# CVMI-Lab/HybridNeuralRendering

Hardware: AMD Instinct MI355X
Metric: rays/sec (fwd render) scene0241_01 at 1/2/4/8 GPU; PSNR delta vs ref (higher is better)
Workload: dtype f32

## Files before the change

### hybridneuralrendering_amd/csrc/chain_ws.hip

```cpp
#include <utility>

#include "chain_defs.h"
#include "hnr_launch.h"

namespace hnr {

constexpr int CW_CST = ch_lds_exch(4) + 2048;
constexpr int CW_CST_FLOATS = CH_META_DESCALE + 4;
constexpr int CW_DSUM = CW_CST + ((CW_CST_FLOATS * 4 + 15) & ~15);
constexpr int CW_HMAX = CW_DSUM + 4 * 32 * 4 * 4;
constexpr int cw_lds_bytes() { return CW_HMAX + 5 * 512; }

#define CW_LOAD_FRAG(N_, rsrc_, voff_, soff_, IMM_) asm volatile("buffer_load_dwordx4 a[%2:%3], %0, %1, %4 offen offset:%5" :: "v"(voff_), "s"(rsrc_), "n"(N_), "n"((N_) + 3), "s"(soff_), "n"(IMM_))
template <int N> __device__ __forceinline__ void cw_mfma(f32x16 &acc, const u32x4 &x)
{
    asm volatile("v_mfma_f32_32x32x16_f16 %0, a[%2:%3], %1, %0" : "+v"(acc) : "v"(x), "n"(N), "n"(N + 3));
}
template <int N> __device__ __forceinline__ void cw_mfma_first(f32x16 &acc, const u32x4 &x)
{
    asm volatile("v_mfma_f32_32x32x16_f16 %0, a[%2:%3], %1, 0" : "=&v"(acc) : "v"(x), "n"(N), "n"(N + 3));
}
__device__ __forceinline__ void cw_mfma_vw(f32x16 &acc, const u32x4 &w, const u32x4 &x)
{
    asm volatile("v_mfma_f32_32x32x16_f16 %0, %1, %2, %0" : "+v"(acc) : "v"(w), "v"(x));
// ... 31 lines not shown
}

template <class F, int... Is> __device__ __forceinline__ void cw_static_seq(F &&f, std::integer_sequence<int, Is...>) { (f(std::integral_constant<int, Is>{}), ...); }
template <int N, class F> __device__ __forceinline__ void cw_static_for(F &&f) { cw_static_seq(f, std::make_integer_sequence<int, N>{}); }

constexpr int cw_steps(int L) { return L == 0 ? CH_S0 : L == 1 ? CH_S1 : L == 2 ? CH_S2 : CH_S3; }
constexpr int cw_korder(int L, int i) { return L == 1 ? ((i + 8) & 15) : i; }
constexpr int cw_wbase(int L) { return L == 0 ? CH_W0 : L == 1 ? CH_W1 : L == 2 ? CH_W2 : CH_W3; }
constexpr int cw_goff(int P) { int g = 0; for (int p = 0; p < P; ++p) g += cw_steps(p >> 2); return g; }
constexpr int CW_GTOT = cw_goff(16);

constexpr int cw_issue(int P, int slot)
{
    const int L = P >> 2, rt = P & 3;
    if (L == 0) {
        if (rt == 0) return slot == 14 ? 32 + 12 : slot == 20 ? 32 + 13 : -1;
        if (rt == 1) return slot == 17 ? 32 + 14 : -1;
        if (rt == 2) return slot == 17 ? 32 + 15 : -1;
        return -1;
    }
    if (slot % 6 != 5) return -1;
    const int it = slot / 6;
    if (P == 4) return it < 8 ? 32 + it : -1;
    if (P == 7) {
        const int t[16] = {-1, -1, 8, -1, -1, 9, -1, -1, 0, 1, -1, 2, 3, -1, 4, 5};
        return t[it] < 0 ? -1 : 64 + t[it];
    }
    if (P == 8) { const int t[17] = {6, 7, 10, 11, -1, 12, -1, 13, -1, 14, 15, -1, -1, -1, -1, -1, -1}; return t[it] < 0 ? -1 : 64 + t[it]; }
    if (P == 11) return (it & 1) && it < 16 ? 96 + (it >> 1) : -1;
    if (P == 12) { const int t[16] = {8, 9, 10, -1, 11, 12, -1, 13, 14, -1, 15, -1, -1, -1, -1, -1}; return t[it] < 0 ? -1 : 96 + t[it]; }
    if (P == 15) return it < 4 ? it : (it >= 8 && it < 12) ? 32 + it : -1;
    return -1;
}
constexpr int cw_stamp(int P, int slot, int ph) { return (P * 128 + slot) * 4 + ph; }
constexpr int CW_TILE_STAMPS = 16 * 128 * 4;
constexpr int cw_train_stores(int P, int sl)
{
    const int S = cw_steps(P >> 2), T = 6 * S, H = T / 2;
    const bool wide = S == 4;
    int n = 0;
    if (sl < H) {
        const int MS = wide ? 17 : 33, PLe = ((P + 15) & 15) >> 2;
        for (int ms = sl * MS / H; ms < (sl + 1) * MS / H; ++ms) {
            if (wide) { if (ms == 15) n += 4; }
            else if (ms == 23 || ms == 25) n += 2;
            if (ms == MS - 1 && PLe != 3) n += 1;
        }
    } else {
        const int PLe = ((P + 15) & 15) >> 2, MS2 = PLe != 3 ? 21 : 35, k2 = sl - H, N2 = T - H;
        for (int ms = k2 * MS2 / N2; ms < (k2 + 1) * MS2 / N2; ++ms)
            if (ms == 4 || ms == 5) n += 2;
    }
    return n;
}
constexpr int cw_train_stores_pass(int P) { int n = 0; for (int sl = 0; sl < 6 * cw_steps(P >> 2); ++sl) n += cw_train_stores(P, sl); return n; }
static_assert(cw_train_stores_pass(0) == 8 && cw_train_stores_pass(4) == 9 && cw_train_stores_pass(5) == 9 && cw_train_stores_pass(9) == 9 && cw_train_stores_pass(15) == 8, "eight activation stores per pass (+ the sign word of a hidden layer's row tile)");
constexpr int cw_asm_between(int t0, int t1, bool trn = false)
{
    int n = 0;
    for (int wrap = -1; wrap <= 0; ++wrap)
        for (int Q = 0; Q < 16; ++Q)
            for (int sl = 0; sl < 6 * cw_steps(Q >> 2); ++sl) {
                if (cw_issue(Q, sl) >= 0) { const int t = cw_stamp(Q, sl, 2) + wrap * CW_TILE_STAMPS; if (t > t0 && t < t1) n += 4; }
                if ((Q >> 2) == 3 && sl == 3 * cw_steps(3)) { const int t = cw_stamp(Q, sl, 0) + wrap * CW_TILE_STAMPS; if (t > t0 && t < t1) n += 2; }
                if (trn && cw_train_stores(Q, sl) > 0) { const int t = cw_stamp(Q, sl, 3) + wrap * CW_TILE_STAMPS; if (t > t0 && t < t1) n += cw_train_stores(Q, sl); }
            }
    return n;
}
constexpr int cw_need_count(int blk, int P, int slot, bool trn = false)
{
    const int t_need = cw_stamp(P, slot, 1);
    int t_blk = -2 * CW_TILE_STAMPS;
    for (int wrap = -1; wrap <= 0; ++wrap)
        for (int Q = 0; Q < 16; ++Q)
            for (int sl = 0; sl < 6 * cw_steps(Q >> 2); ++sl)
                if (cw_issue(Q, sl) == blk) { const int t = cw_stamp(Q, sl, 2) + wrap * CW_TILE_STAMPS; if (t < t_need && t > t_blk) t_blk = t; }
    return cw_asm_between(t_blk, t_need, trn);
}
constexpr int cw_dma_count(int rt, int Pw, bool trn = false)
{
    const int t1 = cw_stamp(Pw, 3 * cw_steps(Pw >> 2), 0);
    int t0 = cw_stamp(12 + rt, 48, 0);
    if (t0 >= t1) t0 -= CW_TILE_STAMPS;
    return cw_asm_between(t0, t1, trn);
}
static_assert(cw_need_count(32 + 0, 4, 48) == 28 && cw_need_count(32 + 7, 4, 90) == 0, "block1.2's k steps 0..7 are fetched behind the first eight iterations of pass (1,0)");
static_assert(cw_need_count(3, 0, 18) == 22 && cw_need_count(0, 0, 0) == 30, "layer 0 fetches: followed by the image DMA of row tile 3, block1.2's 8..11, then by the first fetch of pass (0,0)");
static_assert(cw_dma_count(3, 2) == 28 && cw_dma_count(0, 15) >= 16, "image DMA waits");

__device__ __forceinline__ void cw_halves(float x, float &lo, float &hi)
{
    const auto r = __builtin_amdgcn_permlane32_swap(__float_as_uint(x), __float_as_uint(x), false, false);
    lo = __uint_as_float(r[0]); hi = __uint_as_float(r[1]);
}
typedef float cw_f32x4 __attribute__((ext_vector_type(4)));
template <class T> using cw_lptr = __attribute__((address_space(3))) T *;
template <int DBG>
__global__ __launch_bounds__(256, 1) void chain_ws_kernel(ChainArgs a)
{
    constexpr bool TR = DBG == 8;
    constexpr int DB = TR ? 0 : DBG;
    constexpr int SLOT = ch_slot(4);
    extern __shared__ __attribute__((aligned(16))) char lds[];
    const int tid = threadIdx.x, lane = tid & 63, wave = __builtin_amdgcn_readfirstlane(tid >> 6), h = lane >> 5, j = lane & 31;
    const ChainClasses cls = chain_classes(a.counts, a.cap_samples);
    const int n_valid = cls.n_valid, n_tiles = cls.n_tiles;
    const float *meta = reinterpret_cast<const float *>(a.wimg + CH_META);
    const __amdgpu_buffer_rsrc_t wsrd = __builtin_amdgcn_make_buffer_rsrc(const_cast<char *>(a.wimg), 0, CH_WBYTES, 0x00020000);
    const int col0 = 64 * wave + 16 * h;
    const unsigned woff = (unsigned)(2 * wave) * 2048u + (unsigned)lane * 16u;
    const int o_b0 = (int)lane * 16, o_b1 = o_b0 + 65536, o_b2 = o_b0 + 131072;
    const int o_pub = (int)(4 * wave + h) * SLOT + (int)j * 16;
    const int o_ext = 16 * SLOT + (int)j * 16;
    const int o_exw = (int)ch_lds_exch(4) + (int)(j * 4 + wave) * 4, o_exr = (int)ch_lds_exch(4) + (int)j * 16;
    const int o_dsw = (int)CW_DSUM + (int)(j * 4 + wave) * 4, o_dsr = (int)CW_DSUM + (int)wave * 512 + (int)j * 16;
    const int o_cst = (int)CW_CST + (int)col0 * 4;
#define CW_KEEP(x_) ({ int k_ = (x_); asm volatile("" : "+v"(k_)); k_; })
#define CW_LDS(T_, off_) (*reinterpret_cast<T_ *>(lds + (off_)))
#define CW_AT(T_, ptr_, off_) (*reinterpret_cast<cw_lptr<T_>>((ptr_) + (off_)))
// ... 9 lines not shown
        if constexpr (pe_ != 3) { q_pub = CW_KEEPP(p_pub); q_exw = CW_KEEPP(p_exw); q_exr = CW_KEEPP(p_exr); } \
        if constexpr (pe_ == 1) q_ext = CW_KEEPP(p_ext); \
        if constexpr (pe_ == 3) { q_dsw = CW_KEEPP(p_dsw); q_dsr = CW_KEEPP(p_dsr); } } while (0)

    const int xcd = blockIdx.x & 7, nb = (gridDim.x + 7 - xcd) / 8, bi = blockIdx.x >> 3;
    const int per = (n_tiles + 7) / 8, t_lo = xcd * per, t_hi = (t_lo + per < n_tiles) ? t_lo + per : n_tiles;
    const bool xcd_order = gridDim.x >= 8;
    const int t_first = xcd_order ? t_lo + bi : (int)blockIdx.x, t_end = xcd_order ? t_hi : n_tiles, t_step = xcd_order ? nb : (int)gridDim.x;
    if (t_first >= t_end) return;

    for (int i = tid; i < 2 * 4 * 32; i += 256)
        CW_LDS(u32x4, 16 * SLOT + (i >> 5) * 1024 + (32 + (i & 31)) * 16) = u32x4{0u, 0u, 0u, 0u};
    for (int i = tid; i < CW_CST_FLOATS; i += 256) CW_LDS(float, CW_CST + 4 * i) = meta[i];
    if constexpr (TR) { for (int i = tid; i < 5 * 128; i += 256) CW_LDS(float, CW_HMAX + 4 * i) = 0.f; }

    asm volatile("" ::: "a255");
    u32x4 wx[2][2];
    f32x16 acc[2][2];
    u32x4 bf[3][2];
    float inv[4] = {0.f, 0.f, 0.f, 0.f};
    int pid[4], pid_n[4] = {0, 0, 0, 0};
    float wq[4], wq_fin = 0.f;
    float4 e0 = make_float4(0.f, 0.f, 0.f, 0.f), e1 = e0;
    float4 tv[TR ? 1 : 2][2][4];
#define CW_TV(i_) tv[TR ? 0 : ((i_) & 1)]

#ifndef HNR_CHAIN_WS_SAME_W
#define HNR_CHAIN_WS_SAME_W 0
#endif
#define CW_LOAD_W(L_, s_) do { \
        const int so_ = cw_wbase(L_) + (HNR_CHAIN_WS_SAME_W ? 0 : (s_)) * CH_WSTEP; \
        CW_LOAD_FRAG(16 * (s_) + 0, wsrd, woff, so_, 0); CW_LOAD_FRAG(16 * (s_) + 4, wsrd, woff, so_, 1024); \
        CW_LOAD_FRAG(16 * (s_) + 8, wsrd, woff, so_, 2048); CW_LOAD_FRAG(16 * (s_) + 12, wsrd, woff, so_, 3072); } while (0)
    auto load_ids = [&](int tile, int (&pd)[4]) __attribute__((always_inline)) {
        const char *aux = a.aux + (size_t)tile * 4 * CH_AUX_GROUP;
#pragma unroll
        for (int rt = 0; rt < 4; ++rt) {
            if constexpr (TR) { const int u = a.row_u[(size_t)tile * 128 + 32 * rt + j]; pd[rt] = (unsigned)u >= (unsigned)a.ucap ? 0 : u; }
            else pd[rt] = reinterpret_cast<const int32_t *>(aux + rt * CH_AUX_GROUP)[j];
        }
    };
    auto load_rest = [&](int tile) __attribute__((always_inline)) {
        const char *aux = a.aux + (size_t)tile * 4 * CH_AUX_GROUP;
#pragma unroll
        for (int rt = 0; rt < 4; ++rt) wq[rt] = reinterpret_cast<const float *>(aux + rt * CH_AUX_GROUP + 128)[j];
        e0 = *reinterpret_cast<const float4 *>(aux + wave * CH_AUX_GROUP + 256 + j * 32);
        e1 = *reinterpret_cast<const float4 *>(aux + wave * CH_AUX_GROUP + 256 + j * 32 + 16);
    };
    auto load_table = [&](int pr, float4 (&t)[2][4]) __attribute__((always_inline)) {
        const int tq = j & 3;
        const int p0 = __builtin_amdgcn_update_dpp(0, pr, 0x00, 0xf, 0xf, false), p1 = __builtin_amdgcn_update_dpp(0, pr, 0x55, 0xf, 0xf, false),
                  p2 = __builtin_amdgcn_update_dpp(0, pr, 0xAA, 0xf, 0xf, false), p3 = __builtin_amdgcn_update_dpp(0, pr, 0xFF, 0xf, 0xf, false);
        const int pp[4] = {p0, p1, p2, p3};
#pragma unroll
        for (int r = 0; r < 4; ++r) {
            const float *trow = a.ptab + (size_t)(pp[r] < 0 ? 0 : pp[r]) * a.ldt + col0 + 4 * (r ^ tq);
#pragma unroll
            for (int cc = 0; cc < 2; ++cc) t[cc][r] = *reinterpret_cast<const float4 *>(trow + 32 * cc);
        }
    };
    const unsigned lds_base = (unsigned)reinterpret_cast<uintptr_t>(lds);
    const int dma_voff = lane * 16;
    auto dma_image = [&](int tile, int rt) __attribute__((always_inline)) {
        const char *g = a.xp + ((size_t)tile * 4 + rt) * CH_XP_GROUP + wave * 1024;
        const unsigned l0 = lds_base + (unsigned)((wave >> 1) * SLOT + (wave & 1) * 1024 + rt * 2048);
        cw_dma_image(g, g + 4096, dma_voff, l0, l0 + 2 * SLOT);
// ... 53 lines not shown
    float x5_flag = 1.f, x5_flag2 = 1.f;
    float kf[2][4] = {{0.f, 0.f, 0.f, 0.f}, {0.f, 0.f, 0.f, 0.f}};
    float4 ex4 = make_float4(0.f, 0.f, 0.f, 0.f);

    auto read_cst = [&](int L4, int k) __attribute__((always_inline)) {
        return (DB == 5 || DB == 7) ? make_float4(a.slope, 1.f, a.slope, 1.f) : CW_AT_F4(q_cst, L4 * 1024 + (k >> 2) * 128 + (k & 3) * 16);
    };
    auto tr_group = [&](int PL, int PR, int c, int sub, const TileOut &to) __attribute__((always_inline)) {
        const int se = PR & 1;
        auto dppx = [&](float v, int x) __attribute__((always_inline)) -> float {
            const int i = __builtin_bit_cast(int, v);
            const int r = x == 1 ? __builtin_amdgcn_update_dpp(0, i, 0xB1, 0xf, 0xf, false) : x == 2 ? __builtin_amdgcn_update_dpp(0, i, 0x4E, 0xf, 0xf, false)
                                                                                             : __builtin_amdgcn_update_dpp(0, i, 0x1B, 0xf, 0xf, false);
            return __builtin_bit_cast(float, r);
        };
        if (sub == 0) {
            tb[0] = make_float4(acc[se][c][0], acc[se][c][1], acc[se][c][2], acc[se][c][3]);
            tb[1] = make_float4(dppx(acc[se][c][4], 1), dppx(acc[se][c][5], 1), dppx(acc[se][c][6], 1), dppx(acc[se][c][7], 1));
        } else if (sub == 1) {
            tb[2] = make_float4(dppx(acc[se][c][8], 2), dppx(acc[se][c][9], 2), dppx(acc[se][c][10], 2), dppx(acc[se][c][11], 2));
            tb[3] = make_float4(dppx(acc[se][c][12], 3), dppx(acc[se][c][13], 3), dppx(acc[se][c][14], 3), dppx(acc[se][c][15], 3));
        } else if (sub == 2) cw_table_swap(tb[0], tb[1], tb[2], tb[3]);
        else {
            const int ld4 = a.ldh[PL] * 4;
            const int sb = (to.t < 0 ? (int)0x80000000 : (to.t * 128 + 32 * PR) * ld4 + wave * 256) + 128 * c;
            const int jj = CW_KEEP(j);
            const int hvq = (jj & ~3) * ld4 + (CW_KEEP(h) * 64 + sb), t16 = (jj & 3) * 16;
#pragma unroll
            for (int r = 2 * (sub - 3); r < 2 * (sub - 3) + 2; ++r)
                __builtin_amdgcn_raw_buffer_store_b128(u32x4{__float_as_uint(tb[r].x), __float_as_uint(tb[r].y), __float_as_uint(tb[r].z), __float_as_uint(tb[r].w)}, hrs[PL],
                                                       hvq + r * ld4 + ((16 * r) ^ t16), 0, 0);
        }
    };
    auto epilogue_piece = [&](int PL, int PR, int S, int slot, const TileOut &to) __attribute__((always_inline)) {
        const int T = 6 * S, H = T / 2, se = PR & 1;
        const int exb = (PR & 1) * 512;
        const float inv_l = PL == 0 ? inv0 : inv[PR];
        const int PLn = PR == 3 ? (PL + 1) & 3 : PL;
        if (slot < H) {
            auto fh_st0 = [&](int it, float &o_x, float &o_y, float &o_a, float &o_b) __attribute__((always_inline)) {
                const int c = it >> 3, q = it & 7, k = it >> 1;
                if (it == 0) { amax = 0.f; ap = 0.f; }
                if ((it & 1) == 0 && k >= 1 && k + 1 < 8) { bq[(k + 1) & 1] = read_cst(PL, k + 1); if (PL == 3) aq[(k + 1) & 1] = read_cst(4, k + 1); }
                float ax = (it & 1) ? bq[k & 1].z : bq[k & 1].x, ay = (it & 1) ? bq[k & 1].w : bq[k & 1].y;
                if (PL == 0) {
                    if (q == 0) cw_table_swap(CW_TV(PR)[c][0], CW_TV(PR)[c][1], CW_TV(PR)[c][2], CW_TV(PR)[c][3]);
                    const float4 t4 = CW_TV(PR)[c][q >> 1];
                    if ((q >> 1) == 0) { ax = cw_table_add<0>((q & 1) ? t4.z : t4.x, ax); ay = cw_table_add<0>((q & 1) ? t4.w : t4.y, ay); }
                    else if ((q >> 1) == 1) { ax = cw_table_add<1>((q & 1) ? t4.z : t4.x, ax); ay = cw_table_add<1>((q & 1) ? t4.w : t4.y, ay); }
                    else if ((q >> 1) == 2) { ax = cw_table_add<2>((q & 1) ? t4.z : t4.x, ax); ay = cw_table_add<2>((q & 1) ? t4.w : t4.y, ay); }
                    else { ax = cw_table_add<3>((q & 1) ? t4.z : t4.x, ax); ay = cw_table_add<3>((q & 1) ? t4.w : t4.y, ay); }
                }
                o_x = fmaf(acc[se][c][2 * q], inv_l, ax); o_y = fmaf(acc[se][c][2 * q + 1], inv_l, ay);
                o_a = __fmul_rn(o_x, a.slope); o_b = __fmul_rn(o_y, a.slope);
            };
            auto fh_st1 = [&](int it, float i_x, float i_y, float i_a, float i_b) __attribute__((always_inline)) {
                const int c = it >> 3, q = it & 7, k = it >> 1;
                const float vx = fmaxf(i_x, i_a), vy = fmaxf(i_y, i_b);
                acc[se][c][2 * q] = vx; acc[se][c][2 * q + 1] = vy;
                if (PL == 3) { ap = fmaf(vx, (it & 1) ? aq[k & 1].z : aq[k & 1].x, ap); ap = fmaf(vy, (it & 1) ? aq[k & 1].w : aq[k & 1].y, ap); }
                else amax = fmaxf(fmaxf(amax, fabsf(vx)), fabsf(vy));
                if constexpr (TR) {
                    if (PL == 3) amax = fmaxf(fmaxf(amax, fabsf(vx)), fabsf(vy));
                    else {
                        unsigned long long cy;
                        asm volatile("v_cmp_gt_f32 vcc, %2, 0\n\tv_cmp_gt_f32_e64 %1, %3, 0\n\tv_addc_co_u32 %0, vcc, %0, %0, vcc\n\tv_addc_co_u32_e64 %0, %1, %0, %0, %1"
                                     : "+v"(mbits), "=&s"(cy) : "v"(vx), "v"(vy) : "vcc");
                    }
                }
                if (DB == 1) {
                    if (a.dbg && a.dbg_layer == PL && to.t >= 0) {
                        int te = to.t;
                        asm volatile("" : "+s"(te));
                        float *o = a.dbg + ((size_t)te * 128 + 32 * PR + j) * 256 + col0 + 32 * c + 2 * q;
                        o[0] = vx; o[1] = vy;
                    }
                }
            };
            const bool wide = S == 4;
            const int MS = wide ? 17 : 33, m0 = slot * MS / H, m1 = (slot + 1) * MS / H;
#pragma unroll
            for (int ms = m0; ms < m1; ++ms) {
                if (ms < MS - 1) {
                    if (wide) {
                        const int i0 = 2 * (ms >> 1), st = ms & 1;
                        if (st == 0) { fh_st0(i0, s1x, s1y, s1a, s1b); fh_st0(i0 + 1, s2x, s2y, s2a, s2b); }
                        else { fh_st1(i0, s1x, s1y, s1a, s1b); fh_st1(i0 + 1, s2x, s2y, s2a, s2b); }
                    } else {
                        if ((ms & 1) == 0) fh_st0(ms >> 1, s1x, s1y, s1a, s1b); else fh_st1(ms >> 1, s1x, s1y, s1a, s1b);
                    }
                } else {
                    float m;
                    float v_lo, v_hi;
                    if (PL == 3) {
                        cw_halves(ap, v_lo, v_hi); m = __fadd_rn(v_lo, v_hi); CW_AT(float, q_dsw, PR * 512) = m;
                        if constexpr (TR) { const float am = __fmul_rn(amax, to.t >= 0 ? 1.f : 0.f); CW_HMAX_PUT(3, am); }
                    }
                    else {
                        cw_halves(amax, v_lo, v_hi);
                        m = fmaxf(v_lo, v_hi);
                        if (PL == 1 && PR == wave)
                            m = fmaxf(m, fmaxf(fmaxf(fmaxf(fabsf(e0.x), fabsf(e0.y)), fmaxf(fabsf(e0.z), fabsf(e0.w))), fmaxf(fmaxf(fabsf(e1.x), fabsf(e1.y)), fabsf(e1.z))));
                    }
                    if (PL != 3 && DB != 6 && DB != 7) CW_AT(float, q_exw, exb) = m;
                    if constexpr (TR) { if (PL != 3) CW_HMAX_PUT(PL, m); }
                    if constexpr (TR) {
                        if (PL != 3)
                            __builtin_amdgcn_raw_buffer_store_b32(mbits, brs, CW_KEEP(lane) * 4, (int)(PL * a.hbits_stride * 4) + ((to.t * 4 + PR) * 4 + wave) * 256, 0);
                    }
                }
                if constexpr (TR) {
                    if (wide) {
                        if (ms == 9) tr_group(PL, PR, 0, 0, to);
                        if (ms == 11) tr_group(PL, PR, 0, 1, to);
                        if (ms == 13) tr_group(PL, PR, 0, 2, to);
                        if (ms == 15) { tr_group(PL, PR, 0, 3, to); tr_group(PL, PR, 0, 4, to); }
                    } else if (ms >= 17 && ms <= 25 && (ms & 1)) tr_group(PL, PR, 0, (ms - 17) >> 1, to);
                }
            }
            return;
        }
        const int k2 = slot - H, N2 = T - H;
        auto prefetch_next = [&]() __attribute__((always_inline)) {
            bq[0] = read_cst(PLn, 0); bq[1] = read_cst(PLn, 1);
            if (PLn == 3) { aq[0] = read_cst(4, 0); aq[1] = read_cst(4, 1); }
        };
        if (PL != 3) {
            const int MS = 21, m0 = k2 * MS / N2, m1 = (k2 + 1) * MS / N2;
#pragma unroll
            for (int ms = m0; ms < m1; ++ms) {
                if constexpr (TR) { if (ms >= 1 && ms <= 5) tr_group(PL, PR, 1, ms - 1, to); }
                if (ms == 0) ex4 = (DB == 5 || DB == 7) ? make_float4(amax, 1.f, 2.f, 3.f) : CW_AT_F4(q_exr, exb);
                else if (ms == 1) {
                    const int k = row_scale_exp(fmaxf(fmaxf(ex4.x, ex4.y), fmaxf(ex4.z, ex4.w)));
                    sc_run = pow2f(k);
                    inv[PR] = __fmul_rn(pow2f(-k), PL == 0 ? dw1 : PL == 1 ? dw2 : dw3);
                } else if (ms < 19) {
                    const int it = ms - 2, ip = it - 1;
                    if (it == 0) {
                        asm volatile("v_fma_mixlo_f16 %0, %1, %3, 0\n\ts_nop 0\n\tv_fma_mixhi_f16 %0, %2, %3, 0"
                                     : "=&v"(ph[0]) : "v"(acc[se][0][0]), "v"(acc[se][0][1]), "v"(sc_run));
                    } else if (it < 16) {
                        const int c = it >> 3, q = it & 7, cp = ip >> 3, qp = ip & 7;
                        asm volatile("v_fma_mixlo_f16 %0, %2, %6, 0\n\t"
                                     "v_fma_mixlo_f16 %1, %4, %6, -%7 op_sel_hi:[0,0,1]\n\t"
                                     "v_fma_mixhi_f16 %0, %3, %6, 0\n\t"
                                     "v_fma_mixhi_f16 %1, %5, %6, -%7 op_sel:[0,0,1] op_sel_hi:[0,0,1]"
                                     : "=&v"(ph[q]), "=&v"(pm[qp])
                                     : "v"(acc[se][c][2 * q]), "v"(acc[se][c][2 * q + 1]), "v"(acc[se][cp][2 * qp]), "v"(acc[se][cp][2 * qp + 1]), "v"(sc_run), "v"(ph[qp]));
                    } else {
                        asm volatile("v_fma_mixlo_f16 %0, %1, %3, -%4 op_sel_hi:[0,0,1]\n\ts_nop 0\n\tv_fma_mixhi_f16 %0, %2, %3, -%4 op_sel:[0,0,1] op_sel_hi:[0,0,1]"
                                     : "=&v"(pm[7]) : "v"(acc[se][1][14]), "v"(acc[se][1][15]), "v"(sc_run), "v"(ph[7]));
                    }
                    if (it < 16 && ((it & 3) == 3) && !(DB == 6 || DB == 7)) {
                        const int c = it >> 3, q = it & 7;
                        CW_AT(u32x4, q_pub, c * 2 * SLOT + PR * 2048 + (q == 7 ? 512 : 0)) = u32x4{ph[q - 3], ph[q - 2], ph[q - 1], ph[q]};
                    }
                    if (ip >= 0) {
                        const int cp = ip >> 3, qp = ip & 7;
                        if ((qp == 3 || qp == 7) && (DB == 6 || DB == 7)) { asm volatile("" :: "v"(ph[qp]), "v"(pm[qp]), "v"(ph[qp - 1]), "v"(pm[qp - 1]), "v"(ph[qp - 2]), "v"(pm[qp - 2]), "v"(ph[qp - 3]), "v"(pm[qp - 3])); }
                        else if (qp == 3 || qp == 7)
                            CW_AT(u32x4, q_pub, cp * 2 * SLOT + PR * 2048 + (qp == 7 ? 512 : 0) + 1024) = u32x4{pm[qp - 3], pm[qp - 2], pm[qp - 1], pm[qp]};
                    }
                } else if (ms == 19) {
                    if (PL == 1 && PR == wave && h == 0) {
                        unsigned xh[4], xm[4];
                        split2h(__fmul_rn(e0.x, sc_run), __fmul_rn(e0.y, sc_run), xh[0], xm[0]);
                        split2h(__fmul_rn(e0.z, sc_run), __fmul_rn(e0.w, sc_run), xh[1], xm[1]);
                        split2h(__fmul_rn(e1.x, sc_run), __fmul_rn(e1.y, sc_run), xh[2], xm[2]);
                        split2h(__fmul_rn(e1.z, sc_run), 0.f, xh[3], xm[3]);
                        CW_AT(u32x4, q_ext, PR * 2048) = u32x4{xh[0], xh[1], xh[2], xh[3]};
                        CW_AT(u32x4, q_ext, PR * 2048 + 1024) = u32x4{xm[0], xm[1], xm[2], xm[3]};
                        if constexpr (TR) {
                            const int ev = ((to.t * 128 + 32 * PR + CW_KEEP(j)) * a.ldh[1] + 256) * 4;
                            __builtin_amdgcn_raw_buffer_store_b128(u32x4{__float_as_uint(e0.x), __float_as_uint(e0.y), __float_as_uint(e0.z), __float_as_uint(e0.w)}, hrs[1], ev, 0, 0);
                            __builtin_amdgcn_raw_buffer_store_b128(u32x4{__float_as_uint(e1.x), __float_as_uint(e1.y), __float_as_uint(e1.z), 0u}, hrs[1], ev + 16, 0, 0);
                        }
                    }
                } else prefetch_next();
            }
            return;
        }
        const float wq_e = PR == 3 ? wq_fin : wq[PR];
        const int kc_e = to.kc;
        const int MS = 35, m0 = k2 * MS / N2, m1 = (k2 + 1) * MS / N2;
#pragma unroll
        for (int ms = m0; ms < m1; ++ms) {
            if constexpr (TR) { if (ms >= 1 && ms <= 5) tr_group(PL, PR, 1, ms - 1, to); }
            if (ms == 0) {
                if (PR == 3) ex4 = CW_AT_F4(q_dsr, 0);
                const int ls = (j >> (3 - kc_e)) + (4 << kc_e) * PR;
                const bool st = (j & ((8 >> kc_e) - 1)) == 0;
                x5_voff = st ? (ls * a.ld5 + col0) * 4 : 0x40000000;
                x5_flag = kc_e > 0 ? 0.f : 1.f;
                x5_flag2 = kc_e > 1 ? 0.f : 1.f;
                if constexpr (TR) x5m = 0.f;
                if constexpr (TR) x5_take = (st && to.first + CW_KEEP(ls) < to.end) ? 1.f : 0.f;
            } else if (ms < 33) {
                const int d = (ms - 1) >> 2, t = (ms - 1) & 3, c = d >> 2, e0i = 4 * (d & 3), kb = d & 1;
                if (t == 0)
                    asm volatile("v_mul_f32 %0, %4, %8\n\tv_mul_f32 %1, %5, %8\n\tv_mul_f32 %2, %6, %8\n\tv_mul_f32 %3, %7, %8"
                                 : "=&v"(kf[kb][0]), "=&v"(kf[kb][1]), "=&v"(kf[kb][2]), "=&v"(kf[kb][3])
                                 : "v"(acc[se][c][e0i]), "v"(acc[se][c][e0i + 1]), "v"(acc[se][c][e0i + 2]), "v"(acc[se][c][e0i + 3]), "v"(wq_e));
                else if (t == 1)
                    asm volatile("v_add_f32_dpp %0, %0, %0 quad_perm:[1,0,3,2] row_mask:0xf bank_mask:0xf\n\tv_add_f32_dpp %1, %1, %1 quad_perm:[1,0,3,2] row_mask:0xf bank_mask:0xf\n\t"
                                 "v_add_f32_dpp %2, %2, %2 quad_perm:[1,0,3,2] row_mask:0xf bank_mask:0xf\n\tv_add_f32_dpp %3, %3, %3 quad_perm:[1,0,3,2] row_mask:0xf bank_mask:0xf"
                                 : "+v"(kf[kb][0]), "+v"(kf[kb][1]), "+v"(kf[kb][2]), "+v"(kf[kb][3]));
                else if (t == 2)
                    asm volatile("v_fmac_f32_dpp %0, %0, %4 quad_perm:[2,3,0,1] row_mask:0xf bank_mask:0xf\n\tv_fmac_f32_dpp %1, %1, %4 quad_perm:[2,3,0,1] row_mask:0xf bank_mask:0xf\n\t"
                                 "v_fmac_f32_dpp %2, %2, %4 quad_perm:[2,3,0,1] row_mask:0xf bank_mask:0xf\n\tv_fmac_f32_dpp %3, %3, %4 quad_perm:[2,3,0,1] row_mask:0xf bank_mask:0xf"
                                 : "+v"(kf[kb][0]), "+v"(kf[kb][1]), "+v"(kf[kb][2]), "+v"(kf[kb][3]) : "v"(x5_flag2));
                else {
                    asm volatile("v_fmac_f32_dpp %0, %0, %4 row_half_mirror row_mask:0xf bank_mask:0xf\n\tv_fmac_f32_dpp %1, %1, %4 row_half_mirror row_mask:0xf bank_mask:0xf\n\t"
                                 "v_fmac_f32_dpp %2, %2, %4 row_half_mirror row_mask:0xf bank_mask:0xf\n\tv_fmac_f32_dpp %3, %3, %4 row_half_mirror row_mask:0xf bank_mask:0xf"
                                 : "+v"(kf[kb][0]), "+v"(kf[kb][1]), "+v"(kf[kb][2]), "+v"(kf[kb][3]) : "v"(x5_flag));
                    __builtin_amdgcn_raw_buffer_store_b128(u32x4{__float_as_uint(kf[kb][0]), __float_as_uint(kf[kb][1]), __float_as_uint(kf[kb][2]), __float_as_uint(kf[kb][3])}, to.rs,
                                                           x5_voff + (32 * c + e0i) * 4, 0, 0);
                    if constexpr (TR) {
// ... 47 lines not shown
            __builtin_amdgcn_sched_barrier(0);
            cw_static_for<6 * S>([&](auto kc) __attribute__((always_inline)) {
                constexpr int slot = decltype(kc)::value, it = slot / 6, s = cw_korder(L, it), g = (slot % 6) >> 1, c = slot & 1;
                if (slot == H) {
                    if constexpr (P == 15) { constexpr int d_ = cw_dma_count(0, 15, TR); if constexpr (d_ <= 63) cw_wait_vm<d_>(); }
                    if constexpr (P == 2) { constexpr int d_ = cw_dma_count(3, 2, TR); if constexpr (d_ <= 63) cw_wait_vm<d_>(); }
                    if (DB >= 2 && P == 1) { const long long t_ = clock64(); tmf[0] += t_ - tf_prev; tf_prev = t_; }
                    cw_lds_barrier();
                    if (DB >= 2 && P == 1) { const long long t_ = clock64(); tmf[1] += t_ - tf_prev; tf_prev = t_; }
                    if constexpr (L == 3) dma_image(tile_nx, rt);
                    if constexpr (!TR && L == 0 && rt < 3) load_table(pid[rt + 1], tv[TR ? 0 : (rt + 1) & 1]);
                    if constexpr (TR && L == 0 && rt >= 1) load_table(pid[rt], tv[0]);
                    if constexpr (P == 14) load_table(pid_n[0], tv[0]);
                    if (DB >= 2 && P == 1) { const long long t_ = clock64(); tmf[2] += t_ - tf_prev; tf_prev = t_; }
                    __builtin_amdgcn_sched_barrier(0);
                }
                constexpr int wp = g == 0 ? 1 : 0, xp_ = g == 1 ? 1 : 0;
                constexpr int ring = (G0 + it) % 3;
                if constexpr (rt == 0 && g == 0 && c == 0 && s < 16) {
                    constexpr int n_ = cw_need_count(32 * L + s, P, slot, TR) + (P == 0 ? 8 : 0);
                    if constexpr (n_ <= (TR ? 63 : 56)) cw_wait_vm<n_>();
                }
                constexpr int A0 = 16 * (s < 16 ? s : 0) + 4 * wp + 8 * c;
                if constexpr (DB == 4) { if (slot < 2) { acc[sm][c] = f32x16{} + bf[ring][xp_][0]; } }
                else if constexpr (L == 2 && s == 16) cw_mfma_vw(acc[sm][c], wx[c][wp], bf[ring][xp_]);
                else if constexpr (slot < 2) cw_mfma_first<A0>(acc[sm][c], bf[ring][xp_]);
                else cw_mfma<A0>(acc[sm][c], bf[ring][xp_]);
                __builtin_amdgcn_sched_barrier(0);
                if constexpr (g < 2 && c == 0 && G0 + it + 2 < CW_GTOT) {
                    constexpr int i2 = it + 2 >= S ? it + 2 - S : it + 2, P2 = it + 2 >= S ? P + 1 : P;
                    if constexpr (P2 < 16 && i2 < cw_steps((P2 & 15) >> 2)) bf[(G0 + it + 2) % 3][g] = b_read(P2 & 3, cw_korder((P2 & 15) >> 2, i2), g);
                }
                if constexpr (g < 2 && c == 0 && P == 15 && it == 15) bf[0][g] = b_read(0, 0, g);
                { constexpr int blk = cw_issue(P, slot); if constexpr (blk >= 0) CW_LOAD_W(blk >> 5, blk & 31); }
                if (DB != 3) epilogue_piece(PL, PR, S, slot, to_e);
                __builtin_amdgcn_sched_barrier(0);
            });
        });
        wq_fin = wq[3]; to_fin = to_cur;
#pragma unroll
        for (int rt = 0; rt < 4; ++rt) pid[rt] = pid_n[rt];
    }
    CW_REFRESH(0);
    cw_static_for<6 * CH_S0>([&](auto kc) __attribute__((always_inline)) {
        constexpr int slot = decltype(kc)::value;
        if (slot == (6 * CH_S0) / 2) cw_lds_barrier();
        epilogue_piece(3, 3, CH_S0, slot, to_fin);
    });
    asm volatile("s_waitcnt vmcnt(0)" ::: "memory");
    if constexpr (TR) {
        __syncthreads();
        float *exch = reinterpret_cast<float *>(lds + ch_lds_exch(4));
#pragma unroll
        for (int l = 0; l < 5; ++l) {
            float m = tid < 128 ? CW_LDS(float, CW_HMAX + l * 512 + 4 * tid) : 0.f;
            for (int o = 32; o > 0; o >>= 1) m = fmaxf(m, __shfl_xor(m, o));
            if (lane == 0) exch[4 * l + wave] = m;
        }
        __syncthreads();
        if (tid < 5) {
            const float m = fmaxf(fmaxf(exch[4 * tid], exch[4 * tid + 1]), fmaxf(exch[4 * tid + 2], exch[4 * tid + 3]));
            unsigned *dst = tid < 4 ? (a.hmax ? a.hmax + tid : nullptr) : a.x5max;
            if (dst && m > 0.f) atomicMax(dst, __float_as_uint(m));
        }
    }
    if (DB >= 2 && blockIdx.x == 0 && lane == 0 && a.dbg) {
        long long *o = reinterpret_cast<long long *>(a.dbg) + 4 * 1024 + wave * 16;
        for (int i = 0; i < 16; ++i) o[i] = tm[i];
        if (wave == 0) { long long *o2 = reinterpret_cast<long long *>(a.dbg) + 4 * 1024 + 64; for (int i = 0; i < 4; ++i) o2[i] = tmf[i]; }
    }
    if (DB >= 2 && tid == 0 && a.dbg) {
        long long *o = reinterpret_cast<long long *>(a.dbg) + 4 * (size_t)blockIdx.x;
        o[0] = clock64() - t_start; o[1] = wall_clock64() - w_start; o[2] = n_my; o[3] = 0;
    }
}

__global__ __launch_bounds__(128) void chain_sigma_kernel(ChainArgs a)
{
    const ChainClasses cls = chain_classes(a.counts, a.cap_samples);
    const int tile = blockIdx.x;
// ... 41 lines not shown
```

Before: 8.147 million.

## Spread weight-fragment loads one per MFMA gap and cost-balance epilogue micro-stage placement

In the long passes, each weight block's four buffer_load_dwordx4 fragments are now issued one per MFMA gap over four consecutive slots instead of all four in one gap. The epilogue micro-stages are placed in slots by a compile-time dynamic program that weighs the estimated cost of each gap, replacing the old even split. The hidden-layer second-half epilogue is also broken into finer micro-stages, including a staged f16 hi/lo split of the extra features. The aim is to smooth issue pressure between MFMAs so each gap fits behind the matrix op; the price is much more constexpr machinery, and the hand-tuned cost model and vmcnt wait counts must stay consistent with the schedule.

```diff
diff --git a/hybridneuralrendering_amd/csrc/chain_ws.hip b/hybridneuralrendering_amd/csrc/chain_ws.hip
--- a/hybridneuralrendering_amd/csrc/chain_ws.hip
+++ b/hybridneuralrendering_amd/csrc/chain_ws.hip
@@ -87,24 +87,129 @@
     if (P == 15) return it < 4 ? it : (it >= 8 && it < 12) ? 32 + it : -1;
     return -1;
 }
+constexpr int cw_load_at(int P, int slot, int j)
+{
+    if ((P >> 2) == 0) return cw_issue(P, slot);
+    int Q = P, sl = slot - j;
+    if (sl < 0) { Q = P - 1; if ((Q >> 2) == 0) return -1; sl += 6 * cw_steps(Q >> 2); }
+    return cw_issue(Q, sl);
+}
+constexpr bool cw_loads_stay_long() { for (int sl = 6 * cw_steps(3) - 3; sl < 6 * cw_steps(3); ++sl) if (cw_issue(15, sl) >= 0) return false; return true; }
+static_assert(cw_loads_stay_long(), "a block fetched behind the last three MFMAs of pass (3,3) would spill into the short pass (0,0)");
+constexpr int cw_loads_behind(int P, int slot) { int n = 0; for (int j = 0; j < 4; ++j) n += cw_load_at(P, slot, j) >= 0 ? 1 : 0; return n; }
+
+constexpr int CW_MS1 = 33, CW_MS1_WIDE = 17;
+constexpr int CW_MS2_HID = 29, CW_MS2_L3 = 35;
+constexpr int CW_MAX_SLOTS = 6 * CH_S2;
+constexpr int cw_ms_count(int PLe, bool second, bool wide) { return !second ? (wide ? CW_MS1_WIDE : CW_MS1) : (PLe == 3 ? CW_MS2_L3 : CW_MS2_HID); }
+constexpr int cw_gap_pre(int P, int sl)
+{
+    const int L = P >> 2, T = 6 * cw_steps(L), H = T / 2, Pn = (P + 1) & 15;
+    int c = 4;
+    if (sl % 6 == 0 || sl % 6 == 2) c += 4;
+    c += 16 * cw_loads_behind(P, sl);
+    if (sl == H - 1) c += 8 + (L == 3 ? 48 : 0);
+    if (sl == T - 1) c += 32 + (Pn == 6 || Pn == 13 || Pn == 1 ? 64 : 0);
+    return c;
+}
+constexpr int cw_ms_cost(int PLe, bool second, int ms)
+{
+    if (!second) {
+        if (ms == CW_MS1 - 1) return PLe == 1 ? 60 : 28;
+        if (ms & 1) return PLe == 3 ? 24 : 12;
+        int c = 16 + (PLe == 0 ? 8 : 0);
+        if ((ms & 3) == 0 && ms >= 4 && ms <= 24) c += PLe == 3 ? 8 : 4;
+        if (PLe == 0 && (ms == 0 || ms == 16)) c += 96;
+        return c;
+    }
+    if (PLe != 3) {
+        if (ms == 0) return 4;
+        if (ms == 1) return 24;
+        if (ms == 2) return 40;
+        if (ms < 20) { const int it = ms - 3; return (it == 0 || it == 16 ? 12 : 16) + ((it & 3) == 3 ? 13 : 0) + (it >= 4 && (it & 3) == 0 ? 13 : 0); }
+        if (ms < 28) return PLe == 1 ? 24 : 0;
+        return 12;
+    }
+    if (ms == 0) return 72;
+    if (ms < 33) return ((ms - 1) & 3) == 3 ? 36 : 16;
+    return ms == 33 ? 28 : 16;
+}
+constexpr int cw_ms_from21(int o) { return o <= 1 ? o : o <= 19 ? o + 1 : o == 20 ? CW_MS2_HID - 1 : CW_MS2_HID; }
+struct CwPlaceRow { unsigned char lo[CW_MAX_SLOTS], hi[CW_MAX_SLOTS]; };
+constexpr CwPlaceRow cw_make_place_row(int P)
+{
+    CwPlaceRow r{};
+    const int S = cw_steps(P >> 2), T = 6 * S, H = T / 2, PLe = ((P + 15) & 15) >> 2;
+    const bool wide = S == CH_S0;
+    for (int half = 0; half < 2; ++half) {
+        const int MS = cw_ms_count(PLe, half == 1, wide), s0 = half ? H : 0, N = half ? T - H : H;
+        if (wide) {
+            const bool old21 = half == 1 && PLe != 3;
+            const int MSo = old21 ? 21 : MS;
+            for (int k = 0; k < N; ++k) {
+                const int lo = k * MSo / N, hi = (k + 1) * MSo / N;
+                r.lo[s0 + k] = (unsigned char)(old21 ? cw_ms_from21(lo) : lo); r.hi[s0 + k] = (unsigned char)(old21 ? cw_ms_from21(hi) : hi);
+            }
+            continue;
+        }
+        const int a = half ? H : 1, b = half ? T : H - 2, n = b - a;
+        constexpr long long INF = 1ll << 60;
+        long long best[CW_MS2_L3 + 1][CW_MAX_SLOTS / 2 + 2] = {};
+        bool take[CW_MS2_L3 + 1][CW_MAX_SLOTS / 2 + 2] = {};
+        for (int m = 0; m <= MS; ++m)
+            for (int s = 0; s <= n; ++s) {
+                if (m == 0) { best[m][s] = 0; continue; }
+                if (s < m) { best[m][s] = INF; continue; }
+                const int pre = cw_gap_pre(P, a + s - 1), ld = pre + cw_ms_cost(PLe, half == 1, m - 1);
+                const int ov = ld > 32 ? ld - 32 : 0, ov0 = pre > 32 ? pre - 32 : 0;
+                const int d = (a + s - 1) - (a + ((2 * (m - 1) + 1) * n) / (2 * MS));
+                const long long with = best[m - 1][s - 1] + 8ll * (ov * ov - ov0 * ov0) + (ld * ld - pre * pre) + 2ll * d * d, without = best[m][s - 1];
+                take[m][s] = with <= without;
+                best[m][s] = take[m][s] ? with : without;
+            }
+        for (int k = 0; k < N; ++k) { r.lo[s0 + k] = 0; r.hi[s0 + k] = 0; }
+        unsigned char at[CW_MS2_L3] = {};
+        for (int m = MS, s = n; m > 0; --s) if (take[m][s]) { at[m - 1] = (unsigned char)(a + s - 1); --m; }
+        for (int sl = s0, m = 0; sl < s0 + N; ++sl) {
+            r.lo[sl] = (unsigned char)m;
+            if (m < MS && at[m] == sl) ++m;
+            r.hi[sl] = (unsigned char)m;
+        }
+    }
+    return r;
+}
+template <int P> constexpr CwPlaceRow cw_place_row = cw_make_place_row(P);
+struct CwPlace { CwPlaceRow row[16]; };
+constexpr CwPlace cw_place = {{cw_place_row<0>, cw_place_row<1>, cw_place_row<2>, cw_place_row<3>, cw_place_row<4>, cw_place_row<5>, cw_place_row<6>, cw_place_row<7>,
+                               cw_place_row<8>, cw_place_row<9>, cw_place_row<10>, cw_place_row<11>, cw_place_row<12>, cw_place_row<13>, cw_place_row<14>, cw_place_row<15>}};
+constexpr int cw_ms_lo(int P, int sl) { return cw_place.row[P].lo[sl]; }
+constexpr int cw_ms_hi(int P, int sl) { return cw_place.row[P].hi[sl]; }
+constexpr bool cw_place_complete(int P)
+{
+    const int S = cw_steps(P >> 2), T = 6 * S, H = T / 2, PLe = ((P + 15) & 15) >> 2;
+    for (int half = 0; half < 2; ++half) {
+        int m = 0;
+        for (int sl = half ? H : 0; sl < (half ? T : H); ++sl) { if (cw_ms_lo(P, sl) != m || cw_ms_hi(P, sl) < m) return false; m = cw_ms_hi(P, sl); }
+        if (m != cw_ms_count(PLe, half == 1, S == CH_S0)) return false;
+    }
+    return S == CH_S0 || (cw_ms_hi(P, 0) == 0 && cw_ms_lo(P, H - 2) == CW_MS1);
+}
+constexpr bool cw_place_all_complete() { for (int P = 0; P < 16; ++P) if (!cw_place_complete(P)) return false; return true; }
+static_assert(cw_place_all_complete(), "placement table: a micro-stage is missing, doubled or on the wrong side of the barrier");
+
 constexpr int cw_stamp(int P, int slot, int ph) { return (P * 128 + slot) * 4 + ph; }
 constexpr int CW_TILE_STAMPS = 16 * 128 * 4;
 constexpr int cw_train_stores(int P, int sl)
 {
-    const int S = cw_steps(P >> 2), T = 6 * S, H = T / 2;
-    const bool wide = S == 4;
+    const int S = cw_steps(P >> 2), T = 6 * S, H = T / 2, PLe = ((P + 15) & 15) >> 2;
+    const bool wide = S == CH_S0;
     int n = 0;
-    if (sl < H) {
-        const int MS = wide ? 17 : 33, PLe = ((P + 15) & 15) >> 2;
-        for (int ms = sl * MS / H; ms < (sl + 1) * MS / H; ++ms) {
+    for (int ms = cw_ms_lo(P, sl); ms < cw_ms_hi(P, sl); ++ms) {
+        if (sl < H) {
             if (wide) { if (ms == 15) n += 4; }
             else if (ms == 23 || ms == 25) n += 2;
-            if (ms == MS - 1 && PLe != 3) n += 1;
-        }
-    } else {
-        const int PLe = ((P + 15) & 15) >> 2, MS2 = PLe != 3 ? 21 : 35, k2 = sl - H, N2 = T - H;
-        for (int ms = k2 * MS2 / N2; ms < (k2 + 1) * MS2 / N2; ++ms)
-            if (ms == 4 || ms == 5) n += 2;
+            if (ms == (wide ? CW_MS1_WIDE : CW_MS1) - 1 && PLe != 3) n += 1;
+        } else if (ms == 4 || ms == 5) n += 2;
     }
     return n;
 }
@@ -116,7 +221,7 @@
     for (int wrap = -1; wrap <= 0; ++wrap)
         for (int Q = 0; Q < 16; ++Q)
             for (int sl = 0; sl < 6 * cw_steps(Q >> 2); ++sl) {
-                if (cw_issue(Q, sl) >= 0) { const int t = cw_stamp(Q, sl, 2) + wrap * CW_TILE_STAMPS; if (t > t0 && t < t1) n += 4; }
+                if (cw_loads_behind(Q, sl) > 0) { const int t = cw_stamp(Q, sl, 2) + wrap * CW_TILE_STAMPS; if (t > t0 && t < t1) n += cw_loads_behind(Q, sl); }
                 if ((Q >> 2) == 3 && sl == 3 * cw_steps(3)) { const int t = cw_stamp(Q, sl, 0) + wrap * CW_TILE_STAMPS; if (t > t0 && t < t1) n += 2; }
                 if (trn && cw_train_stores(Q, sl) > 0) { const int t = cw_stamp(Q, sl, 3) + wrap * CW_TILE_STAMPS; if (t > t0 && t < t1) n += cw_train_stores(Q, sl); }
             }
@@ -129,9 +234,28 @@
     for (int wrap = -1; wrap <= 0; ++wrap)
         for (int Q = 0; Q < 16; ++Q)
             for (int sl = 0; sl < 6 * cw_steps(Q >> 2); ++sl)
-                if (cw_issue(Q, sl) == blk) { const int t = cw_stamp(Q, sl, 2) + wrap * CW_TILE_STAMPS; if (t < t_need && t > t_blk) t_blk = t; }
+                if (cw_load_at(Q, sl, 3) == blk) { const int t = cw_stamp(Q, sl, 2) + wrap * CW_TILE_STAMPS; if (t < t_need && t > t_blk) t_blk = t; }
     return cw_asm_between(t_blk, t_need, trn);
 }
+constexpr bool cw_loads_before_need()
+{
+    int n = 0;
+    for (int Q = 0; Q < 16; ++Q)
+        for (int sl = 0; sl < 6 * cw_steps(Q >> 2); ++sl)
+            for (int j = 0; j < 4; ++j) {
+                const int blk = cw_load_at(Q, sl, j);
+                if (blk < 0) continue;
+                const int L = blk >> 5, s = blk & 31;
+                int it = 0;
+                for (int i = 0; i < cw_steps(L); ++i) if (cw_korder(L, i) == s) it = i;
+                int dt = cw_stamp(4 * L, 6 * it, 1) - cw_stamp(Q, sl, 2);
+                if (dt < 0) dt += CW_TILE_STAMPS;
+                if (dt > CW_TILE_STAMPS / 2) return false;
+                ++n;
+            }
+    return n == 4 * (CH_S0 + CH_S1 + 16 + CH_S3);
+}
+static_assert(cw_loads_before_need(), "a weight block's four loads are not all out when its layer's first pass waits for it");
 constexpr int cw_dma_count(int rt, int Pw, bool trn = false)
 {
     const int t1 = cw_stamp(Pw, 3 * cw_steps(Pw >> 2), 0);
@@ -139,7 +263,8 @@
     if (t0 >= t1) t0 -= CW_TILE_STAMPS;
     return cw_asm_between(t0, t1, trn);
 }
-static_assert(cw_need_count(32 + 0, 4, 48) == 28 && cw_need_count(32 + 7, 4, 90) == 0, "block1.2's k steps 0..7 are fetched behind the first eight iterations of pass (1,0)");
+static_assert(cw_need_count(32 + 0, 4, 48) == 25 && cw_need_count(32 + 7, 4, 90) == 0, "block1.2's k steps 0..7 are fetched behind the first eight iterations of pass (1,0), one load per MFMA");
+static_assert(cw_loads_behind(4, 5) == 1 && cw_loads_behind(4, 8) == 1 && cw_loads_behind(4, 9) == 0 && cw_loads_behind(8, 0) == 1 && cw_loads_behind(0, 14) == 4, "one load per gap in the long passes (pass (1,3)'s last block ends in pass (2,0)), four in the short ones");
 static_assert(cw_need_count(3, 0, 18) == 22 && cw_need_count(0, 0, 0) == 30, "layer 0 fetches: followed by the image DMA of row tile 3, block1.2's 8..11, then by the first fetch of pass (0,0)");
 static_assert(cw_dma_count(3, 2) == 28 && cw_dma_count(0, 15) >= 16, "image DMA waits");
 
@@ -215,6 +340,9 @@
         const int so_ = cw_wbase(L_) + (HNR_CHAIN_WS_SAME_W ? 0 : (s_)) * CH_WSTEP; \
         CW_LOAD_FRAG(16 * (s_) + 0, wsrd, woff, so_, 0); CW_LOAD_FRAG(16 * (s_) + 4, wsrd, woff, so_, 1024); \
         CW_LOAD_FRAG(16 * (s_) + 8, wsrd, woff, so_, 2048); CW_LOAD_FRAG(16 * (s_) + 12, wsrd, woff, so_, 3072); } while (0)
+#define CW_LOAD_W1(L_, s_, j_) do { \
+        const int so_ = cw_wbase(L_) + (HNR_CHAIN_WS_SAME_W ? 0 : (s_)) * CH_WSTEP; \
+        CW_LOAD_FRAG(16 * (s_) + 4 * (j_), wsrd, woff, so_, 1024 * (j_)); } while (0)
     auto load_ids = [&](int tile, int (&pd)[4]) __attribute__((always_inline)) {
         const char *aux = a.aux + (size_t)tile * 4 * CH_AUX_GROUP;
 #pragma unroll
@@ -334,7 +462,7 @@
                                                        hvq + r * ld4 + ((16 * r) ^ t16), 0, 0);
         }
     };
-    auto epilogue_piece = [&](int PL, int PR, int S, int slot, const TileOut &to) __attribute__((always_inline)) {
+    auto epilogue_piece = [&](int PL, int PR, int S, int slot, int m0, int m1, const TileOut &to) __attribute__((always_inline)) {
         const int T = 6 * S, H = T / 2, se = PR & 1;
         const int exb = (PR & 1) * 512;
         const float inv_l = PL == 0 ? inv0 : inv[PR];
@@ -380,7 +508,7 @@
                 }
             };
             const bool wide = S == 4;
-            const int MS = wide ? 17 : 33, m0 = slot * MS / H, m1 = (slot + 1) * MS / H;
+            const int MS = wide ? CW_MS1_WIDE : CW_MS1;
 #pragma unroll
             for (int ms = m0; ms < m1; ++ms) {
                 if (ms < MS - 1) {
@@ -422,23 +550,22 @@
             }
             return;
         }
-        const int k2 = slot - H, N2 = T - H;
         auto prefetch_next = [&]() __attribute__((always_inline)) {
             bq[0] = read_cst(PLn, 0); bq[1] = read_cst(PLn, 1);
             if (PLn == 3) { aq[0] = read_cst(4, 0); aq[1] = read_cst(4, 1); }
         };
         if (PL != 3) {
-            const int MS = 21, m0 = k2 * MS / N2, m1 = (k2 + 1) * MS / N2;
 #pragma unroll
             for (int ms = m0; ms < m1; ++ms) {
                 if constexpr (TR) { if (ms >= 1 && ms <= 5) tr_group(PL, PR, 1, ms - 1, to); }
                 if (ms == 0) ex4 = (DB == 5 || DB == 7) ? make_float4(amax, 1.f, 2.f, 3.f) : CW_AT_F4(q_exr, exb);
-                else if (ms == 1) {
-                    const int k = row_scale_exp(fmaxf(fmaxf(ex4.x, ex4.y), fmaxf(ex4.z, ex4.w)));
+                else if (ms == 1) ex4.x = fmaxf(fmaxf(ex4.x, ex4.y), fmaxf(ex4.z, ex4.w));
+                else if (ms == 2) {
+                    const int k = row_scale_exp(ex4.x);
                     sc_run = pow2f(k);
                     inv[PR] = __fmul_rn(pow2f(-k), PL == 0 ? dw1 : PL == 1 ? dw2 : dw3);
-                } else if (ms < 19) {
-                    const int it = ms - 2, ip = it - 1;
+                } else if (ms < 20) {
+                    const int it = ms - 3, ip = it - 1;
                     if (it == 0) {
                         asm volatile("v_fma_mixlo_f16 %0, %1, %3, 0\n\ts_nop 0\n\tv_fma_mixhi_f16 %0, %2, %3, 0"
                                      : "=&v"(ph[0]) : "v"(acc[se][0][0]), "v"(acc[se][0][1]), "v"(sc_run));
@@ -464,15 +591,23 @@
                         else if (qp == 3 || qp == 7)
                             CW_AT(u32x4, q_pub, cp * 2 * SLOT + PR * 2048 + (qp == 7 ? 512 : 0) + 1024) = u32x4{pm[qp - 3], pm[qp - 2], pm[qp - 1], pm[qp]};
                     }
-                } else if (ms == 19) {
-                    if (PL == 1 && PR == wave && h == 0) {
-                        unsigned xh[4], xm[4];
-                        split2h(__fmul_rn(e0.x, sc_run), __fmul_rn(e0.y, sc_run), xh[0], xm[0]);
-                        split2h(__fmul_rn(e0.z, sc_run), __fmul_rn(e0.w, sc_run), xh[1], xm[1]);
-                        split2h(__fmul_rn(e1.x, sc_run), __fmul_rn(e1.y, sc_run), xh[2], xm[2]);
-                        split2h(__fmul_rn(e1.z, sc_run), 0.f, xh[3], xm[3]);
-                        CW_AT(u32x4, q_ext, PR * 2048) = u32x4{xh[0], xh[1], xh[2], xh[3]};
-                        CW_AT(u32x4, q_ext, PR * 2048 + 1024) = u32x4{xm[0], xm[1], xm[2], xm[3]};
+                } else if (ms < 28) {
+                    const int e = (ms - 20) >> 1;
+                    if (PL == 1 && PR == wave) {
+                        if (((ms - 20) & 1) == 0) {
+                            s1x = __fmul_rn(e == 0 ? e0.x : e == 1 ? e0.z : e == 2 ? e1.x : e1.z, sc_run);
+                            s1y = e == 3 ? 0.f : __fmul_rn(e == 0 ? e0.y : e == 1 ? e0.w : e1.y, sc_run);
+                            asm("v_cvt_pk_f16_f32 %0, %1, %2" : "=v"(ph[e]) : "v"(s1x), "v"(s1y));
+                        } else {
+                            float r0, r1;
+                            asm("v_fma_mix_f32 %0, -%1, 1.0, %2 op_sel_hi:[1,0,0]" : "=v"(r0) : "v"(ph[e]), "v"(s1x));
+                            asm("v_fma_mix_f32 %0, -%1, 1.0, %2 op_sel:[1,0,0] op_sel_hi:[1,0,0]" : "=v"(r1) : "v"(ph[e]), "v"(s1y));
+                            asm("v_cvt_pk_f16_f32 %0, %1, %2" : "=v"(pm[e]) : "v"(r0), "v"(r1));
+                        }
+                    }
+                    if (ms == 27 && PL == 1 && PR == wave && h == 0) {
+                        CW_AT(u32x4, q_ext, PR * 2048) = u32x4{ph[0], ph[1], ph[2], ph[3]};
+                        CW_AT(u32x4, q_ext, PR * 2048 + 1024) = u32x4{pm[0], pm[1], pm[2], pm[3]};
                         if constexpr (TR) {
                             const int ev = ((to.t * 128 + 32 * PR + CW_KEEP(j)) * a.ldh[1] + 256) * 4;
                             __builtin_amdgcn_raw_buffer_store_b128(u32x4{__float_as_uint(e0.x), __float_as_uint(e0.y), __float_as_uint(e0.z), __float_as_uint(e0.w)}, hrs[1], ev, 0, 0);
@@ -485,7 +620,6 @@
         }
         const float wq_e = PR == 3 ? wq_fin : wq[PR];
         const int kc_e = to.kc;
-        const int MS = 35, m0 = k2 * MS / N2, m1 = (k2 + 1) * MS / N2;
 #pragma unroll
         for (int ms = m0; ms < m1; ++ms) {
             if constexpr (TR) { if (ms >= 1 && ms <= 5) tr_group(PL, PR, 1, ms - 1, to); }
@@ -599,8 +733,12 @@
                     if constexpr (P2 < 16 && i2 < cw_steps((P2 & 15) >> 2)) bf[(G0 + it + 2) % 3][g] = b_read(P2 & 3, cw_korder((P2 & 15) >> 2, i2), g);
                 }
                 if constexpr (g < 2 && c == 0 && P == 15 && it == 15) bf[0][g] = b_read(0, 0, g);
-                { constexpr int blk = cw_issue(P, slot); if constexpr (blk >= 0) CW_LOAD_W(blk >> 5, blk & 31); }
-                if (DB != 3) epilogue_piece(PL, PR, S, slot, to_e);
+                cw_static_for<4>([&](auto jc) __attribute__((always_inline)) {
+                    constexpr int j_ = decltype(jc)::value, blk = cw_load_at(P, slot, j_);
+                    if constexpr (blk >= 0) CW_LOAD_W1(blk >> 5, blk & 31, j_);
+                });
+                constexpr int m0_ = cw_ms_lo(P, slot), m1_ = cw_ms_hi(P, slot);
+                if (DB != 3) epilogue_piece(PL, PR, S, slot, m0_, m1_, to_e);
                 __builtin_amdgcn_sched_barrier(0);
             });
         });
@@ -612,7 +750,8 @@
     cw_static_for<6 * CH_S0>([&](auto kc) __attribute__((always_inline)) {
         constexpr int slot = decltype(kc)::value;
         if (slot == (6 * CH_S0) / 2) cw_lds_barrier();
-        epilogue_piece(3, 3, CH_S0, slot, to_fin);
+        constexpr int m0_ = cw_ms_lo(0, slot), m1_ = cw_ms_hi(0, slot);
+        epilogue_piece(3, 3, CH_S0, slot, m0_, m1_, to_fin);
     });
     asm volatile("s_waitcnt vmcnt(0)" ::: "memory");
     if constexpr (TR) {
```

Result: no change. 8.209 million (median of 6 runs) (+0.8%).
